# leoelm/Bayesian_inference_for_NN

Measured on AMD Instinct MI355X. Metric: posterior samples/sec (grad-steps/sec) on MLP 784->200->10, batch 1024, higher is better.
Workload: dtype f32; 1 GPU; SGLD, MLP 784->200->10 (D=159010), synthetic MNIST-shaped 48000x784 fp32 resident in HBM, batch 1024 (last batch of an epoch 896), 1 chain per GPU, device-resident run replayed from hipGraphs; seed=2024, parallelism=independent chains x1 (replicas only, no data-path collective)

## Files before the change

bayesian_inference_for_nn_amd/csrc/pyz_api.hip:

```cpp

#include <algorithm>
#include <cmath>
#include <cstring>

#include "pyz_common.h"
#include "pyz_fused.h"
#include "pyz_gemm.h"
#include "pyz_gemm_ring.h"
#include "pyz_hmc_fused.h"
#include "pyz_hmc_multi.h"
#include "pyz_input_grad.h"
#include "pyz_kernels.h"
#include "pyz_predict_moments.h"
#include "pyz_rng.h"
#include "pyz_sgld_chains.h"

namespace {

inline hipStream_t as_stream(void *s) { return reinterpret_cast<hipStream_t>(s); }
inline int cdiv(long long a, long long b) { return (int)((a + b - 1) / b); }

int ensure_bytes(void **ptr, size_t *cap, size_t need, pyz_mlp *m) {
  if (*cap >= need) return PYZ_OK;
  if (*ptr) PYZ_HIP(hipFree(*ptr));
  *ptr = nullptr;
  *cap = 0;
  PYZ_HIP(hipMalloc(ptr, need));
  m->ws_bytes += need;
  *cap = need;
  return PYZ_OK;
}

struct Extra {
  size_t grad_cap = 0, grad2_cap = 0, qsave_cap = 0, part_cap = 0, part2_cap = 0, scal_cap = 0;
// ... 321 lines not shown
    g.ctl = ctl;
    pyz_launch_bwd_data(g, grid_batch, P, st);
  }
}

inline int wgrad_tiles(const pyz_mlp *m) {
  int tiles = 0;
  for (int l = 0; l < m->L; ++l) tiles += ((m->dims[l] + 1 + 31) / 32) * ((m->dims[l + 1] + 31) / 32);
  return tiles;
}

int wgrad_layers(pyz_mlp *m, int P, const float *x, const int32_t *row_idx, const StepCtl *ctl, WgradArgs &a,
                 const float *gathered) {
  int tiles = 0;
  a.L = m->L;
  for (int l = 0; l < m->L; ++l) {
    WgradLayer &ly = a.lay[l];
    ly.K = m->dims[l];
    ly.N = m->dims[l + 1];
    if (l == 0) {
      ly.in = (row_idx && gathered) ? gathered : x;
      ly.in_pstride = 0;
      ly.gather = (row_idx && !gathered) ? 1 : 0;
    } else {
      ly.in = m->act[l - 1];
      ly.in_pstride = (long long)m->max_batch * ly.K;
      ly.gather = 0;
    }
    ly.lda = ly.K;
    ly.delta = m->delta[l];
    ly.delta_pstride = (long long)m->max_batch * ly.N;
    ly.w_off = m->w_off[l];
    ly.tile0 = tiles;
    tiles += ((ly.K + 1 + 31) / 32) * ((ly.N + 31) / 32);
  }
  a.row_idx = row_idx;
  a.ctl = ctl;
  a.part = m->part;
  a.nblk = m->cur_nblk;
  a.tiles = tiles;
  a.nonfinite = m->nonfinite;
  a.wt = pyz_wt_for(P);
  return tiles;
}

void launch_wgrad_all(pyz_mlp *m, int P, const float *x, const int32_t *row_idx, int grid_batch, const StepCtl *ctl,
                      WgradArgs &a, hipStream_t st, const float *gathered) {
  const int tiles = wgrad_layers(m, P, x, row_idx, ctl, a, gathered);
  const int S = pyz_pick_waves((long long)tiles * P, (grid_batch + 1) / 2);
  dim3 grid(pyz_pad8((long long)tiles + 1, P), P);
  if (a.prep.src && P == 1) grid.x = (unsigned)(tiles + 1 + std::max(pyz_cu_count() - tiles - 1, 24));
  switch (S) {
    case 1:
      if (a.mode == PYZ_UPD_NONE) PYZ_LAUNCH((k_wgrad_all<1, true>), grid, dim3(64), 0, st, a);
      else PYZ_LAUNCH(k_wgrad_all<1>, grid, dim3(64), 0, st, a);
      break;
    case 2: PYZ_LAUNCH(k_wgrad_all<2>, grid, dim3(128), 2 * 4096, st, a); break;
    case 4: PYZ_LAUNCH(k_wgrad_all<4>, grid, dim3(256), 4 * 4096, st, a); break;
    case 8: PYZ_LAUNCH(k_wgrad_all<8>, grid, dim3(512), 8 * 4096, st, a); break;
    default: PYZ_LAUNCH(k_wgrad_all<16>, grid, dim3(1024), 16 * 4096, st, a); break;
  }
}

void launch_wgrad_adam(pyz_mlp *m, const float *x, const int32_t *row_idx, int grid_batch, const StepCtl *ctl, AdamArgs &a,
                       hipStream_t st, const float *gathered) {
  const int tiles = wgrad_layers(m, 1, x, row_idx, ctl, a.w, gathered);
  const int S = pyz_pick_waves(tiles, (grid_batch + 1) / 2);
  const dim3 grid(tiles + 1);
// ... 2367 lines not shown
```

bayesian_inference_for_nn_amd/csrc/pyz_common.h:

```cpp
#pragma once

#include <hip/hip_runtime.h>
#include <hip/hip_ext.h>

#include <cstdarg>
#include <cstdint>
#include <cstdio>
#include <string>
#include <vector>

#include "../../include/pyz.h"

#define PYZ_MAX_LAYERS 16

typedef float f32x16 __attribute__((ext_vector_type(16)));
typedef float f32x4 __attribute__((ext_vector_type(4)));

struct StepCtl {
  int32_t batch;
  float lr;
  long long n;
  long long row_off;
  int32_t i;
  int32_t slot0;
// ... 2 lines not shown

#ifdef PYZ_STAMPS
#define PYZ_STAMP_KERNELS 6
#define PYZ_STAMP_BLOCKS 256
#define PYZ_STAMP_WAVES 16
#define PYZ_STAMP_SLOTS 8
__device__ unsigned long long pyz_dbg_buf[PYZ_STAMP_KERNELS][PYZ_STAMP_BLOCKS][PYZ_STAMP_WAVES][PYZ_STAMP_SLOTS][2];
#define PYZ_STAMP(kid, slot)                                                                   \
  do {                                                                                         \
    __builtin_amdgcn_sched_barrier(0);                                                         \
    if ((threadIdx.x & 63) == 0 && blockIdx.x < PYZ_STAMP_BLOCKS && blockIdx.y == 0) {        \
      unsigned long long t0_, t1_;                                                             \
      asm volatile("s_memtime %0\n\ts_memrealtime %1\n\ts_waitcnt lgkmcnt(0)" : "=s"(t0_), "=s"(t1_)::"memory"); \
      pyz_dbg_buf[kid][blockIdx.x][threadIdx.x >> 6][slot][0] = t0_;                          \
      pyz_dbg_buf[kid][blockIdx.x][threadIdx.x >> 6][slot][1] = t1_;                          \
    }                                                                                          \
    __builtin_amdgcn_sched_barrier(0);                                                         \
  } while (0)
#define PYZ_LAP(lap, slot)                                                                   \
  do {                                                                                       \
    __builtin_amdgcn_sched_barrier(0);                                                       \
    unsigned long long t_;                                                                   \
    asm volatile("s_memtime %0\n\ts_waitcnt lgkmcnt(0)" : "=s"(t_)::"memory");              \
    (lap)[slot] += t_ - (lap)[15];                                                           \
    (lap)[15] = t_;                                                                          \
    __builtin_amdgcn_sched_barrier(0);                                                       \
  } while (0)
#else
#define PYZ_STAMP(kid, slot)
#define PYZ_LAP(lap, slot)
#endif

__device__ __forceinline__ int pyz_wave_id() { return __builtin_amdgcn_readfirstlane((int)(threadIdx.x >> 6)); }

__device__ __forceinline__ StepCtl pyz_ctl_first(const StepCtl *ctl, const StepCtl &init, const int on) {
  if (on && blockIdx.x == 0 && blockIdx.y == 0 && threadIdx.x == 0) *const_cast<StepCtl *>(ctl) = init;
  int ib = init.batch, ii = init.i, is0 = init.slot0, inr = init.n_run;
  float il = init.lr;
  long long in_ = init.n, iro = init.row_off;
  asm volatile("" : "+s"(ib), "+s"(ii), "+s"(is0), "+s"(il), "+s"(in_), "+s"(iro), "+s"(inr));
  StepCtl c;
  c.batch = on ? ib : ctl->batch;
  c.lr = on ? il : ctl->lr;
  c.n = on ? in_ : ctl->n;
  c.row_off = on ? iro : ctl->row_off;
  c.i = on ? ii : ctl->i;
  c.slot0 = on ? is0 : ctl->slot0;
  c.n_run = on ? inr : ctl->n_run;
  return c;
}

__device__ __forceinline__ void pyz_st(float *p, const float v, const int wt) {
  if (wt)
    asm volatile("global_store_dword %0, %1, off sc1" ::"v"(p), "v"(v) : "memory");
  else
    *p = v;
}

inline std::string &pyz_err_slot() {
  static thread_local std::string s;
  return s;
}

inline int pyz_fail(int code, const char *fmt, ...) {
  char buf[512];
  va_list ap;
// ... 147 lines not shown
```

bayesian_inference_for_nn_amd/csrc/pyz_fused.h:

```cpp
#pragma once

#include <type_traits>

#include "pyz_common.h"
#include "pyz_gemm.h"
#include "pyz_kernels.h"

struct HeadArgs {
  const float *hin;
  long long hin_pstride;
  int lda;
  const int32_t *row_idx;
  int gather_hin;
  const float *theta;
  long long theta_pstride;
  long long w_off;
  int K, N;
  int loss, act_last, act_prev, vec;
  const void *y;
  float *out_last;
  float *delta_last;
  float *delta_prev;
  long long last_pstride, prev_pstride;
  double *part;
  int nblk;
  const StepCtl *ctl;
  StepCtl init;
  int init_on;
  int wt;
  const StepCtl *gate;
  int gate_mod;
  const float *hparts;
  int n_hparts;
  long long hpart_stride;
  const float *bias_prev;
  float *h_store;
};

__device__ __forceinline__ float pyz_grp8_max(float v) {
  v = fmaxf(v, __shfl_xor(v, 1, 64));
  v = fmaxf(v, __shfl_xor(v, 2, 64));
  return fmaxf(v, __shfl_xor(v, 4, 64));
}
__device__ __forceinline__ float pyz_grp8_sum(float v) {
  v += __shfl_xor(v, 1, 64);
  v += __shfl_xor(v, 2, 64);
  return v + __shfl_xor(v, 4, 64);
}

__global__ void __launch_bounds__(512) k_head(HeadArgs g) {
  extern __shared__ float lds[];
  PYZ_STAMP(1, 0);
  const int S = blockDim.x >> 6, w = pyz_wave_id(), l = threadIdx.x & 63, r = l & 31, h = l >> 5;
  if (g.gate && g.gate->n % g.gate_mod == 0) return;
  float *red = lds, *zt = lds + S * 1024, *dt = zt + 32 * 33;
  double *lsum = reinterpret_cast<double *>(dt + 32 * 33);
  const StepCtl ctl = pyz_ctl_first(g.ctl, g.init, g.init_on);
  const int batch = ctl.batch, p = blockIdx.y, m0 = blockIdx.x * 32;
  if (m0 >= batch) {
    if (threadIdx.x == 0) g.part[p * g.nblk + blockIdx.x] = 0.0;
    return;
  }
  const int K = g.K, N = g.N;
  const int32_t *idx = g.row_idx ? g.row_idx + ctl.row_off : nullptr;
// ... 179 lines not shown
  return v;
}

__device__ __forceinline__ float pyz_row16_allmax(float v) {
  v = fmaxf(v, pyz_dpp<0xB1>(v));
  v = fmaxf(v, pyz_dpp<0x4E>(v));
  v = fmaxf(v, pyz_dpp<0x141>(v));
  v = fmaxf(v, pyz_dpp<0x140>(v));
  return v;
}

template <int UT, int NP>
struct PyzHeadW {
  float wv[UT][NP];
  float bias_mine;
};

template <int UT, int NP>
__device__ __forceinline__ void pyz_head_load_w(const HeadArgs &g, const int p, const int l, PyzHeadW<UT, NP> &W) {
  const int K = g.K, N = g.N;
  const float *wl = g.theta + p * g.theta_pstride + g.w_off;
  const __amdgpu_buffer_rsrc_t rw = __builtin_amdgcn_make_buffer_rsrc(const_cast<float *>(wl), 0, (K + 1) * N * 4, 0x00020000);
  constexpr unsigned OOB = 0x7FFFFF00u;
#pragma unroll
  for (int t = 0; t < UT; ++t) {
    const int u = l + 64 * t;
    const unsigned wo = u < K ? 4u * (unsigned)u * (unsigned)N : OOB;
#pragma unroll
    for (int c = 0; c < NP; ++c) W.wv[t][c] = pyz_buf_load(rw, wo + 4u * (unsigned)c, 0u);
  }
  W.bias_mine = pyz_buf_load(rw, l < N ? 4u * ((unsigned)K * (unsigned)N + (unsigned)l) : OOB, 0u);
}

template <int UT, int NP, bool PRELOADED, bool HP = false>
__device__ __forceinline__ void pyz_head_row(const HeadArgs &g, const int batch, const long long row_off, const int p,
                                             const int m, const int l, PyzHeadW<UT, NP> &W) {
  const int K = g.K, N = g.N;
  long long yrow = m;
  if (g.row_idx) yrow = g.row_idx[row_off + m];
  const float *hp = g.hin + p * g.hin_pstride + (g.gather_hin ? yrow : (long long)m) * g.lda;
  const __amdgpu_buffer_rsrc_t rh = __builtin_amdgcn_make_buffer_rsrc(const_cast<float *>(hp), 0, K * 4, 0x00020000);
  float hv[UT], z[NP];
  if constexpr (HP) {
    const float *pp = g.hparts + (long long)m * K;
    const __amdgpu_buffer_rsrc_t rp = __builtin_amdgcn_make_buffer_rsrc(const_cast<float *>(pp), 0,
        (int)(((long long)(g.n_hparts - 1) * g.hpart_stride + K) * 4), 0x00020000);
    const __amdgpu_buffer_rsrc_t rb = __builtin_amdgcn_make_buffer_rsrc(const_cast<float *>(g.bias_prev), 0, K * 4, 0x00020000);
    constexpr unsigned OOBH = 0x7FFFFF00u;
    float pv[UT][8], bv[UT];
#pragma unroll
    for (int t = 0; t < UT; ++t) {
      const int u = l + 64 * t;
#pragma unroll
      for (int sp = 0; sp < 8; ++sp)
        pv[t][sp] = pyz_buf_load(rp, (u < K && sp < g.n_hparts) ? 4u * (unsigned)(sp * g.hpart_stride + u) : OOBH, 0u);
      bv[t] = pyz_buf_load(rb, 4u * (unsigned)u, 0u);
    }
#pragma unroll
    for (int t = 0; t < UT; ++t) {
      float a = pv[t][0];
#pragma unroll
      for (int sp = 1; sp < 8; ++sp) a += pv[t][sp];
      hv[t] = pyz_act(a + bv[t], g.act_prev);
      const int u = l + 64 * t;
      if (u < K) pyz_st(g.h_store + (long long)m * K + u, hv[t], g.wt);
    }
  } else {
#pragma unroll
    for (int t = 0; t < UT; ++t) hv[t] = pyz_buf_load(rh, 4u * (unsigned)(l + 64 * t), 0u);
  }
  if (!PRELOADED) pyz_head_load_w<UT, NP>(g, p, l, W);
  const auto &wv = W.wv;
  const float bias_mine = W.bias_mine;
  int ylab = 0;
  if (g.loss == PYZ_LOSS_SCCE) ylab = reinterpret_cast<const int32_t *>(g.y)[yrow];
  PYZ_STAMP(1, 1);
#pragma unroll
  for (int c = 0; c < NP; ++c) {
    float a = 0.0f;
#pragma unroll
    for (int t = 0; t < UT; ++t) a = fmaf(hv[t], wv[t][c], a);
    z[c] = a;
  }
#pragma unroll
  for (int c = 0; c < NP; ++c) {
    const float v = pyz_row16_allsum(z[c]);
    z[c] = ((pyz_readlane(v, 0) + pyz_readlane(v, 16)) + (pyz_readlane(v, 32) + pyz_readlane(v, 48))) + pyz_readlane(bias_mine, c);
  }
  PYZ_STAMP(1, 2);
  float d2[NP], lm, my_d = 0.0f, my_o = 0.0f;
  if (g.loss == PYZ_LOSS_SCCE && NP <= 16) {
    const int lc = l & 15;
    float zc = z[0];
#pragma unroll
    for (int c = 1; c < NP; ++c) zc = (lc == c) ? z[c] : zc;
    const bool on = lc < N;
    const float mx = pyz_row16_allmax(on ? zc : -3.0e38f);
    const float exv = on ? expf(zc - mx) : 0.0f;
    const float se = pyz_row16_allsum(exv);
    const float lse = mx + logf(se);
    const bool mine = on && lc == ylab;
    float zy = pyz_row16_allsum(mine ? zc : 0.0f);
    zy = (ylab >= 0 && ylab < N) ? zy : __builtin_nanf("");
    const float inv = 1.0f / (float)batch, rse = 1.0f / se;
    my_d = (exv * rse - (mine ? 1.0f : 0.0f)) * inv;
    my_o = zc;
// ... 48 lines not shown
      lm = a / (float)N;
    }
#pragma unroll
    for (int c = 0; c < NP; ++c) {
      my_d = (l == c) ? d2[c] : my_d;
      my_o = (l == c) ? outv[c] : my_o;
    }
  }
  PYZ_STAMP(1, 3);
  if (l < N) {
    if (g.out_last) pyz_st(g.out_last + p * g.last_pstride + (long long)m * N + l, my_o, g.wt);
    if (g.delta_last) pyz_st(g.delta_last + p * g.last_pstride + (long long)m * N + l, my_d, g.wt);
  }
  if (l == 0) g.part[p * g.nblk + m] = (double)lm;
  PYZ_STAMP(1, 4);
  if (!g.delta_prev) return;
  float *op = g.delta_prev + p * g.prev_pstride + (long long)m * K;
  const int actp = g.act_prev;
#pragma unroll
  for (int t = 0; t < UT; ++t) {
    const int u = l + 64 * t;
    float a = 0.0f;
#pragma unroll
    for (int c = 0; c < NP; ++c) a = fmaf(d2[c], wv[t][c], a);
    if (u < K) pyz_st(op + u, a * pyz_act_grad(hv[t], actp), g.wt);
  }
  PYZ_STAMP(1, 5);
}

template <int UT, int NP, int RW = 1, bool HP = false>
__global__ void __launch_bounds__(256) k_head_rows(HeadArgs g) {
  PYZ_STAMP(1, 0);
  const int w = pyz_wave_id(), l = threadIdx.x & 63;
  if (g.gate && g.gate->n % g.gate_mod == 0) return;
  const StepCtl ctl = pyz_ctl_first(g.ctl, g.init, g.init_on);
  const int batch = ctl.batch, p = blockIdx.y;
  const int m0 = (blockIdx.x * 4 + w) * RW;
  if (m0 >= batch) {
    if (l < RW && m0 + l < g.nblk) g.part[p * g.nblk + m0 + l] = 0.0;
    return;
  }
  PyzHeadW<UT, NP> W;
  if (RW == 1) {
    pyz_head_row<UT, NP, false, HP>(g, batch, ctl.row_off, p, m0, l, W);
    return;
  }
  pyz_head_load_w<UT, NP>(g, p, l, W);
#pragma unroll 1
  for (int rr = 0; rr < RW; ++rr) {
    const int m = m0 + rr;
    if (m >= batch) {
      if (l == 0 && m < g.nblk) g.part[p * g.nblk + m] = 0.0;
      continue;
    }
    pyz_head_row<UT, NP, true>(g, batch, ctl.row_off, p, m, l, W);
  }
}

struct PrepArgs {
  const float *src;
  float *dst;
  const int32_t *row_idx;
  const int32_t *tab_bs;
  long long row_stride;
  int K, lda;
  int fwd_tiles, fwd_tiles_n;
};

// ... 85 lines not shown
      tab_bc[e] = b.bc[e];
    }
    if (e == 0) {
      ctl->batch = t.bs[0];
      ctl->lr = t.lr[0];
      ctl->n = n;
      ctl->row_off = row_off;
      ctl->i = 0;
      ctl->slot0 = slot0;
      ctl->n_run = t.n - 1;
    }
  }
  pyz_prep_rows(g, g.row_idx + row_off, t.bs[0], (int)blockIdx.x, (int)gridDim.x, (int)blockIdx.x);
}

struct WgradLayer {
  const float *in;
  long long in_pstride;
  const float *delta;
  long long delta_pstride;
  long long w_off;
  int lda, K, N;
  int tile0;
  int gather;
};

#define PYZ_UPD_NONE 0
#define PYZ_UPD_SGD 1
#define PYZ_UPD_SGLD 2
#define PYZ_UPD_BBB 3
#define PYZ_UPD_SWAG 4

struct WgradArgs {
  WgradLayer lay[PYZ_MAX_LAYERS];
  int L;
  int tiles;
  const int32_t *row_idx;
  const StepCtl *ctl;
  int mode;
  float *grad;
  long long grad_pstride;
  float *theta, *mean, *sq_mean;
  uint64_t seed;
  const float *unit_noise;
  float *dev_row;
  int swag_update;
  int swag_freq, swag_k;
  float *dev_base;
  long long dev_stride;
  float alpha, prior_mean, prior_rho, bbb_lr;
  const float *pm_vec, *pr_vec;
  uint32_t bbb_step;
  int bbb_chained;
  const double *part_kl;
  int nblk_kl;
  float *cost;
  float *w_next;
  double *part_kl_next;
  const double *part;
  int nblk;
  float *loss;
  int loss_indexed;
  StepCtl *next;
  const int32_t *tab_bs;
  const float *tab_lr;
  long long row_stride;
  int *nonfinite;
  float *ploss;
  int wt;
  PrepArgs prep;
};

struct PyzUpdOut {
  float th, mu, sq, dev;
  bool wr_mu, wr_sq, wr_dev;
  float *dev_row;
};

__device__ __forceinline__ PyzUpdOut pyz_update_math(const WgradArgs &g, const int mode, const long long e, const float gv,
                                                     const float th0, const float mu0, const float sq0, const float zz,
                                                     const float lr, const long long nstep) {
  PyzUpdOut o;
  o.th = o.mu = o.sq = o.dev = 0.0f;
  o.wr_mu = o.wr_sq = o.wr_dev = false;
  o.dev_row = nullptr;
  if (mode == PYZ_UPD_SGD) {
    o.th = th0 - lr * gv;
  } else if (mode == PYZ_UPD_SWAG) {
    const float th = th0 - lr * gv;
    o.th = th;
    const bool upd = g.swag_freq > 0 ? (nstep % g.swag_freq == 0) : (g.swag_update != 0);
    if (upd) {
      const float fn = (float)nstep, fn1 = fn + 1.0f;
      o.mu = (mu0 * fn + th) / fn1;
      o.sq = (sq0 * fn + th * th) / fn1;
      o.dev = th - o.mu;
      o.wr_mu = o.wr_sq = true;
      o.dev_row = g.swag_freq > 0
                      ? g.dev_base + min((nstep + g.swag_freq - 1) / g.swag_freq, (long long)g.swag_k - 1) * g.dev_stride
                      : g.dev_row;
      o.wr_dev = o.dev_row != nullptr;
    }
  } else if (mode == PYZ_UPD_BBB) {
    const float pmean = g.pm_vec ? g.pm_vec[e] : g.prior_mean;
    const float sp = pyz_softplus(g.pr_vec ? g.pr_vec[e] : g.prior_rho), isp2 = 1.0f / (sp * sp);
    const float mu = th0, rho = mu0, wv = sq0;
    const float sg = pyz_softplus(rho), sig = pyz_sigmoid(rho);
    const float d = wv - mu, is2 = 1.0f / (sg * sg);
    const float g_mu = g.alpha * d * is2;
    const float g_rho = g.alpha * (-1.0f / sg + d * d * is2 / sg) * sig;
    const float g_w = gv + g.alpha * (-d * is2 + (wv - pmean) * isp2);
    const float blr = g.bbb_chained ? lr : g.bbb_lr;
    o.th = mu - blr * (g_mu + g_w);
    o.mu = rho - blr * (zz * sig * g_w + g_rho);
    o.wr_mu = true;
  } else if (mode == PYZ_UPD_SGLD) {
    const float fn = (float)nstep, fn1 = fn + 1.0f;
    const float noise = lr * zz;
    const float th = th0 + (-lr) * (gv + noise);
    o.th = th;
    o.mu = (mu0 * fn + th) / fn1;
    o.sq = (sq0 * fn + th * th) / fn1;
    o.wr_mu = o.wr_sq = true;
  }
  return o;
}

__device__ __forceinline__ void pyz_update_store(const WgradArgs &g, const int mode, const long long e, const int p,
                                                 const float gv, const PyzUpdOut &o) {
  if (mode == PYZ_UPD_NONE) {
    g.grad[p * g.grad_pstride + e] = gv;
    return;
  }
  pyz_st(g.theta + e, o.th, g.wt);
  if (o.wr_mu) pyz_st(g.mean + e, o.mu, g.wt);
  if (o.wr_sq) pyz_st(g.sq_mean + e, o.sq, g.wt);
  if (o.wr_dev) o.dev_row[e] = o.dev;
}

__device__ __forceinline__ void pyz_step_duties(const WgradArgs &g, const int l) {
  const int batch = g.ctl->batch;
  if (g.loss) {
    const double v = pyz_sum_partials(g.part, g.nblk);
    if (l == 0) {
      float *lo = g.loss + (g.loss_indexed ? g.ctl->slot0 + g.ctl->i : 0);
      lo[0] = (float)(v / (double)batch);
      pyz_note_loss(g.nonfinite, lo[0]);
      if (g.next) pyz_prepare_next(g.ctl, g.next, g.tab_bs, g.tab_lr, g.row_stride);
    }
  }
  if (g.mode == PYZ_UPD_BBB) {
    const double v = pyz_sum_partials(g.part, g.nblk), k = pyz_sum_partials(g.part_kl, g.nblk_kl);
    if (l == 0) {
      const float loss = (float)(v / (double)batch), kl = (float)k;
      float *co = g.cost + (g.bbb_chained ? 4 * (g.ctl->slot0 + g.ctl->i) : 0);
// ... 6 lines not shown
  }
}


template <class H>
__device__ __forceinline__ void pyz_wgrad_accumulate(f32x16 &acc, const float *abase, const int ic, const float *dbase,
                                                     const int n, const int lda, const int N, const int batch, int s,
                                                     const int se, const int h, const bool is_w, const bool is_b, H hook) {
  const float bconst = is_b ? 1.0f : 0.0f;
  const unsigned a_lane = ((unsigned)h * (unsigned)lda + (unsigned)ic) * 4u;
  const unsigned d_lane = ((unsigned)h * (unsigned)N + (unsigned)n) * 4u;
  const unsigned a_row2 = 8u * (unsigned)lda, d_row2 = 8u * (unsigned)N;
  const __amdgpu_buffer_rsrc_t ra =
      __builtin_amdgcn_make_buffer_rsrc(const_cast<float *>(abase), 0, (int)((unsigned)batch * (unsigned)lda * 4u), 0x00020000);
  const __amdgpu_buffer_rsrc_t rd =
      __builtin_amdgcn_make_buffer_rsrc(const_cast<float *>(dbase), 0, (int)((unsigned)batch * (unsigned)N * 4u), 0x00020000);
  const int full = batch >> 1;
  pyz_steps1_all(
      s, min(se, full), acc,
      [&](int st, float &a, float &d) {
        a = pyz_buf_load(ra, a_lane, (unsigned)PYZ_HOT(st, batch) * a_row2);
        d = pyz_buf_load(rd, d_lane, (unsigned)PYZ_HOT(st, batch) * d_row2);
      },
      [&](int, float &a, float &) { a = is_w ? a : bconst; }, hook);
  if (se > full) {
    const int b = batch - 1;
    float a = abase[(size_t)b * lda + ic], d = dbase[(size_t)b * N + n];
    a = h == 0 ? (is_w ? a : bconst) : 0.0f;
    d = h == 0 ? d : 0.0f;
    acc = pyz_mfma(a, d, acc);
  }
}

template <int S, bool PLAIN = false>
__global__ void __launch_bounds__(64 * S) k_wgrad_all(WgradArgs g) {
  extern __shared__ float red[];
  PYZ_STAMP(2, 0);
  constexpr int EPT = 16 / S;
  const int w = pyz_wave_id(), l = threadIdx.x & 63;
  const int r = l & 31, h = l >> 5;
  if (blockIdx.x >= (unsigned)g.tiles) {
    if (blockIdx.x == (unsigned)g.tiles && blockIdx.y == 0 && w == 0) pyz_step_duties(g, l);
    if (blockIdx.x == (unsigned)g.tiles && w == 0 && g.ploss) {
      const double tot = pyz_sum_partials(g.part + (long long)blockIdx.y * g.nblk, g.nblk);
      if (l == 0) {
        g.ploss[blockIdx.y] = (float)(tot / (double)g.ctl->batch);
        pyz_note_loss(g.nonfinite, g.ploss[blockIdx.y]);
      }
    }
    if (!PLAIN && blockIdx.x > (unsigned)g.tiles && blockIdx.y == 0 && g.prep.src) {
      const int i2 = g.ctl->i + 1;
      if (i2 < g.ctl->n_run)
        pyz_prep_rows(g.prep, g.prep.row_idx + g.ctl->row_off + g.prep.row_stride, g.prep.tab_bs[i2],
                      (int)blockIdx.x - g.tiles - 1, (int)gridDim.x - g.tiles - 1, (int)blockIdx.x);
      PYZ_STAMP(2, 3);
    }
    return;
  }
  const int tile = pyz_xcd_remap(blockIdx.x, g.tiles);
  int li = 0;
  while (li + 1 < g.L && tile >= g.lay[li + 1].tile0) ++li;
  const WgradLayer &ly = g.lay[li];
  const int batch = g.ctl->batch;
  const int K = ly.K, N = ly.N;
  const int tiles_n = (N + 31) >> 5;
  const int t = tile - ly.tile0;
  const int i0 = (t / tiles_n) * 32, n0 = (t % tiles_n) * 32;
  const int p = blockIdx.y;
  const long long w_off = ly.w_off;
  const int mode = PLAIN ? PYZ_UPD_NONE : g.mode;
  const long long nstep = g.ctl->n;
  const float lr = g.ctl->lr;

  long long ee[EPT];
  bool ev[EPT];
  float th0[PLAIN ? 1 : EPT], mu0[PLAIN ? 1 : EPT], sq0[PLAIN ? 1 : EPT], zz[PLAIN ? 1 : EPT];
  float zg[PLAIN ? 1 : EPT];
  float zn[PLAIN ? 1 : EPT];
  const bool fuse_next = !PLAIN && mode == PYZ_UPD_BBB && g.w_next != nullptr;
  auto prefetch = [&]() {
#pragma unroll
    for (int q = 0; q < EPT; ++q) {
      int ro, co;
      if (S == 1) {
        ro = (q & 3) + 8 * (q >> 2) + 4 * h;
        co = r;
      } else {
        const int e = threadIdx.x + q * 64 * S;
        ro = e >> 5;
        co = e & 31;
      }
      const int ii = i0 + ro, nn = n0 + co;
      ev[q] = ii <= K && nn < N;
      ee[q] = w_off + (long long)min(ii, K) * N + min(nn, N - 1);
      if (PLAIN) continue;
      th0[q] = mu0[q] = sq0[q] = zz[q] = zg[q] = 0.0f;
      if (mode != PYZ_UPD_NONE) th0[q] = g.theta[ee[q]];
      if (mode == PYZ_UPD_SGLD || mode == PYZ_UPD_BBB || mode == PYZ_UPD_SWAG) {
        mu0[q] = g.mean[ee[q]];
        sq0[q] = g.sq_mean[ee[q]];
        if (g.unit_noise && mode != PYZ_UPD_SWAG) zz[q] = g.unit_noise[ee[q]];
      }
    }
    if (!PLAIN && (mode == PYZ_UPD_SGLD || mode == PYZ_UPD_BBB) && !g.unit_noise) {
#pragma unroll
      for (int q = 0; q < EPT; ++q) {
        zg[q] = mode == PYZ_UPD_SGLD ? pyz_normal1(g.seed, PYZ_STREAM_SGLD, (uint32_t)nstep, (uint64_t)ee[q])
                                     : pyz_normal1(g.seed, PYZ_STREAM_BBB, g.bbb_chained ? (uint32_t)nstep : g.bbb_step, (uint64_t)ee[q]);
      }
    }
    if (!PLAIN && fuse_next) {
#pragma unroll
      for (int q = 0; q < EPT; ++q) zn[q] = pyz_normal1(g.seed, PYZ_STREAM_BBB, (uint32_t)(nstep + 1), (uint64_t)ee[q]);
    }
  };

  const int i = i0 + r, n = min(n0 + r, N - 1);
  const int ic = min(i, K - 1);
  const bool is_w = i < K, is_b = i == K;
  const float *ap = ly.in + p * ly.in_pstride + ic;
  const float *dp = ly.delta + p * ly.delta_pstride + n;
  const int32_t *idx = (ly.gather && g.row_idx) ? g.row_idx + g.ctl->row_off : nullptr;
  f32x16 acc = {0};
  const int steps = (batch + 1) >> 1;
  int s = (steps * w) / S;
  const int se = (steps * (w + 1)) / S;
  PYZ_STAMP(2, 1);
  if (idx) {
    prefetch();
    for (int s0 = s; s0 < se; s0 += 32) {
      const int idxv = idx[min(2 * s0 + l, batch - 1)];
      const int lda = ly.lda;
      pyz_steps1_all(
          s0, min(s0 + 32, se), acc,
          [&](int st, float &a, float &d) {
            const int bc = PYZ_HOT(min(2 * st + h, batch - 1), batch);
            const long long row = PYZ_HOT(__shfl(idxv, 2 * (st - s0) + h, 64), batch);
            a = ap[row * lda];
            d = dp[(long long)bc * N];
          },
          [&](int st, float &a, float &d) {
            const bool vb = 2 * st + h < batch;
            a = vb ? (is_w ? a : (is_b ? 1.0f : 0.0f)) : 0.0f;
            d = vb ? d : 0.0f;
          });
    }
  } else {
    pyz_wgrad_accumulate(acc, ly.in + p * ly.in_pstride, ic, ly.delta + p * ly.delta_pstride, n, ly.lda, N, batch, s, se, h,
                         is_w, is_b, prefetch);
  }
  PYZ_STAMP(2, 2);
  float gv[EPT];
  if (S == 1) {
#pragma unroll
    for (int q = 0; q < EPT; ++q) gv[q] = acc[q];
// ... 29 lines not shown
                                        PLAIN ? 0.0f : (g.unit_noise ? zz[q] : zg[q]), lr, nstep);
    pyz_update_store(g, mode, ee[q], p, gv[q], o);
    if (fuse_next) {
      const long long e = ee[q];
      const float pmean = g.pm_vec ? g.pm_vec[e] : g.prior_mean;
      float sp = sp_s, lsp = lsp_s;
      if (g.pr_vec) {
        sp = pyz_softplus(g.pr_vec[e]);
        lsp = logf(sp);
      }
      const float mu = o.th, sg = pyz_softplus(o.mu);
      const float wn = zn[q] * sg + mu;
      pyz_st(g.w_next + e, wn, g.wt);
      const float a = (wn - mu) / sg, b = (wn - pmean) / sp;
      const float lq = -0.5f * a * a - logf(sg) - PYZ_LOG_SQRT_2PI;
      const float lp = -0.5f * b * b - lsp - PYZ_LOG_SQRT_2PI;
      klp += (double)lq - (double)lp;
    }
  }
  if (!PLAIN && fuse_next) {
    double tot = pyz_wave_sum(klp);
    if (S > 1) {
      double *sm = reinterpret_cast<double *>(red);
      __syncthreads();
      if (l == 0) sm[w] = tot;
      __syncthreads();
      tot = 0.0;
      if (threadIdx.x == 0)
        for (int ww = 0; ww < S; ++ww) tot += sm[ww];
    }
    if (threadIdx.x == 0) g.part_kl_next[blockIdx.x] = tot;
  }
  PYZ_STAMP(2, 3);
}

template <class H>
__device__ __forceinline__ void pyz_wgrad_accumulate_sq(f32x16 &acc, f32x16 &acc2, const float fb, const float *abase,
                                                        const int ic, const float *dbase, const int n, const int lda,
                                                        const int N, const int batch, int s, const int se, const int h,
                                                        const bool is_w, const bool is_b, H hook) {
  const float bconst = is_b ? 1.0f : 0.0f;
  const unsigned a_lane = ((unsigned)h * (unsigned)lda + (unsigned)ic) * 4u;
  const unsigned d_lane = ((unsigned)h * (unsigned)N + (unsigned)n) * 4u;
  const unsigned a_row2 = 8u * (unsigned)lda, d_row2 = 8u * (unsigned)N;
  const __amdgpu_buffer_rsrc_t ra =
      __builtin_amdgcn_make_buffer_rsrc(const_cast<float *>(abase), 0, (int)((unsigned)batch * (unsigned)lda * 4u), 0x00020000);
  const __amdgpu_buffer_rsrc_t rd =
      __builtin_amdgcn_make_buffer_rsrc(const_cast<float *>(dbase), 0, (int)((unsigned)batch * (unsigned)N * 4u), 0x00020000);
  const int full = batch >> 1;
  pyz_steps1_all(
      s, min(se, full), acc,
      [&](int st, float &a, float &d) {
        a = pyz_buf_load(ra, a_lane, (unsigned)PYZ_HOT(st, batch) * a_row2);
        d = pyz_buf_load(rd, d_lane, (unsigned)PYZ_HOT(st, batch) * d_row2);
      },
      [&](int, float &a, float &d) {
        a = is_w ? a : bconst;
        const float gd = d * fb;
        acc2 = pyz_mfma(a * a, gd * gd, acc2);
      },
      hook);
  if (se > full) {
    const int b = batch - 1;
    float a = abase[(size_t)b * lda + ic], d = dbase[(size_t)b * N + n];
    a = h == 0 ? (is_w ? a : bconst) : 0.0f;
    d = h == 0 ? d : 0.0f;
// ... 349 lines not shown
```

bayesian_inference_for_nn_amd/csrc/pyz_gemm.h:

```cpp
#pragma once

#include <cstdlib>

#include "pyz_common.h"

struct DenseArgs {
  const float *in;
  long long in_pstride;
  int lda;
  const float *theta;
  long long theta_pstride;
  long long w_off;
  int K, N;
  float *out;
  long long out_pstride;
  const float *aux;
  long long aux_pstride;
  int act;
  int vec;
  const StepCtl *ctl;
  const int32_t *row_idx;
  float *gather_out;
  StepCtl init;
  int init_on;
  int wt;
  int rows_cap;
  int n_part, grid_rows;
  int n_cgrp, cgrp_w;
  int k_split;
  float *part_out;
  long long part_stride;
  const StepCtl *gate;
  int gate_mod;
};

__device__ __forceinline__ int pyz_xcd_remap(const int bid, const int n) {
  const int q = n >> 3, r = n & 7, x = bid & 7, local = bid >> 3;
  return (x < r ? x * (q + 1) : r * (q + 1) + (x - r) * q) + local;
}

#ifdef PYZ_EXP_HOT
#define PYZ_HOT(v, batch) ((v) & ((batch) < 0 ? -1 : 0))
#else
#define PYZ_HOT(v, batch) (v)
#endif

__device__ __forceinline__ f32x16 pyz_mfma(float a, float b, f32x16 c) {
#ifdef PYZ_EXP_NOMFMA
  c[0] += a * b;
  return c;
#else
  return __builtin_amdgcn_mfma_f32_32x32x2f32(a, b, c, 0, 0, 0);
#endif
}

__device__ __forceinline__ float pyz_act(float z, int act) {
  switch (act) {
    case PYZ_ACT_RELU: return z < 0.0f ? 0.0f : z;
    case PYZ_ACT_TANH: return tanhf(z);
    case PYZ_ACT_SIGMOID: return 1.0f / (1.0f + expf(-z));
    default: return z;
  }
}

__device__ __forceinline__ float pyz_act_grad(float h, int act) {
  switch (act) {
    case PYZ_ACT_RELU: return h > 0.0f ? 1.0f : 0.0f;
    case PYZ_ACT_TANH: return 1.0f - h * h;
    case PYZ_ACT_SIGMOID: return h * (1.0f - h);
    default: return 1.0f;
  }
}

__device__ __forceinline__ float pyz_bce_row(float z, float y, float &p) {
  const float e = expf(-fabsf(z));
  const float r = 1.0f / (1.0f + e);
  p = z >= 0.0f ? r : (z < 0.0f ? e * r : z);
  const float u = 1.0f + e;
  const float l1p = u == 1.0f ? e : logf(u) * (e / (u - 1.0f));
  return fmaxf(z, 0.0f) - z * y + l1p;
}

template <class F>
__device__ __forceinline__ void pyz_tile_epilogue(const f32x16 &acc, float *red, F store) {
  const int S = blockDim.x >> 6, w = pyz_wave_id(), l = threadIdx.x & 63;
  const int r = l & 31, h = l >> 5;
  if (S == 1) {
#pragma unroll
    for (int i = 0; i < 16; ++i) store((i & 3) + 8 * (i >> 2) + 4 * h, r, acc[i]);
    return;
  }
  float *my = red + w * 1024;
#pragma unroll
  for (int i = 0; i < 16; ++i) my[((i & 3) + 8 * (i >> 2) + 4 * h) * 32 + r] = acc[i];
  __syncthreads();
  for (int e = threadIdx.x; e < 1024; e += blockDim.x) {
    float s = red[e];
    for (int ww = 1; ww < S; ++ww) s += red[ww * 1024 + e];
    store(e >> 5, e & 31, s);
  }
}

struct PyzNoFix {
  __device__ __forceinline__ void operator()(int, float &, float &) const {}
};

struct PyzNoHook {
  __device__ __forceinline__ void operator()() const {}
};

template <int G, class L, class F, class H = PyzNoHook>
__device__ __forceinline__ void pyz_pipe1(int s, const int se, f32x16 &acc, L load, F fix, H hook = H()) {
  if (s >= se) {
    hook();
    return;
  }
  float an[G], bn[G], a[G], b[G];
  const int last = se - 1;
#pragma unroll
  for (int u = 0; u < G; ++u) load(min(s + u, last), an[u], bn[u]);
  __builtin_amdgcn_sched_barrier(0);
  hook();
  __builtin_amdgcn_sched_barrier(0);
  for (;;) {
#pragma unroll
    for (int u = 0; u < G; ++u) {
      a[u] = an[u];
      b[u] = bn[u];
    }
    const int sn = s + G;
    if (sn < se) {
#pragma unroll
// ... 102 lines not shown
          *reinterpret_cast<float4 *>(gp + 8 * c + 4 * h) = a4;
#endif
        }
      },
      hook);
  const int t0 = 8 * c8, steps = (K - t0 + 1) >> 1;
  const unsigned vt = (unsigned)h * N4 + n4;
  pyz_steps1_all(
      0, (steps - w + S - 1) / S, acc,
      [&](int u, float &a, float &b) {
        const int kb = t0 + 2 * (w + S * u);
        const int kk = kb + h;
        a = ap[kk < K ? kk : 0];
        b = pyz_buf_load(rw, vt, (unsigned)kb * N4);
      },
      [&](int u, float &a, float &b) {
        const int kk = t0 + 2 * (w + S * u) + h;
        const bool vk = kk < K;
        if (gp && vk && copy_rem == 0) gp[kk] = a;
        a = vk ? a : 0.0f;
        b = vk ? b : 0.0f;
      });
  if (w == 0) {
    acc = pyz_mfma(h == 0 ? 1.0f : 0.0f, h == 0 ? bias : 0.0f, acc);
  }
}

__global__ void k_dense_fwd(DenseArgs g) {
  extern __shared__ float red[];
  PYZ_STAMP(0, 0);
  const int S = blockDim.x >> 6, w = pyz_wave_id(), l = threadIdx.x & 63;
  const int r = l & 31, h = l >> 5;
  const int tiles_n = (g.N + 31) >> 5;
  if (g.gate && g.gate->n % g.gate_mod == 0) return;
  const int tile = pyz_xcd_remap(blockIdx.x, gridDim.x);
  const int m0 = (tile / tiles_n) * 32, n0 = (tile % tiles_n) * 32;
  int cap = g.rows_cap;
  long long row_off = 0;
  if (cap <= 0) {
    asm volatile("; the step scalars are needed here" ::: "memory");
    const StepCtl ctl = pyz_ctl_first(g.ctl, g.init, g.init_on);
    cap = __builtin_amdgcn_readfirstlane(ctl.batch);
    row_off = ctl.row_off;
  }
  if (m0 >= cap) return;
  const int p = blockIdx.y;
  const int K = g.K, N = g.N;
  const int m = min(m0 + r, cap - 1), n = min(n0 + r, N - 1);
  long long row = m;
  if (g.row_idx) row = g.row_idx[row_off + m];
  const float *ap = g.in + p * g.in_pstride + row * g.lda;
  const float *wl = g.theta + p * g.theta_pstride + g.w_off;
  f32x16 acc = {0};
  PYZ_STAMP(0, 1);
  float *gp = (g.gather_out && p == 0) ? g.gather_out + (long long)m * K : nullptr;
  int batch = 0;
  const int32_t *ctl_batch = &g.ctl->batch;
  pyz_fwd_accumulate(acc, ap, wl, n, K, N, g.vec, w, S, h, gp, tiles_n, tile % tiles_n,
                     [&]() { batch = __hip_atomic_load(ctl_batch, __ATOMIC_RELAXED, __HIP_MEMORY_SCOPE_AGENT); });
  batch = g.rows_cap > 0 ? __builtin_amdgcn_readfirstlane(batch) : cap;
  PYZ_STAMP(0, 2);
  float *op = g.out + p * g.out_pstride;
  const int act = g.act, wt = g.wt;
  pyz_tile_epilogue(acc, red, [&](int ro, int co, float v) {
    const int mm = m0 + ro, nn = n0 + co;
    if (mm < batch && nn < N) pyz_st(op + (long long)mm * N + nn, pyz_act(v, act), wt);
// ... 372 lines not shown
```

Baseline: 40500 grad-steps/s.

## Reorder kernel arg structs and batch scalar loads to cut kernel prologue latency

Reorders the fields of HeadArgs, DenseArgs and WgradArgs so the hot fields sit together, and uses asm constraints so the compiler issues all kernel-argument scalar loads in one batch at kernel entry. Step-control scalars are now loaded as vector loads and broadcast with readfirstlane. The wgrad layer lookup becomes a branchless compare over a per-layer tile0 table. The update mode is made a template parameter, and the multi-wave tile reduction is unrolled per wave count. These target the fixed prologue and serialized-load latency of small kernels replayed from graphs. The cost is more template instantiations and code size, and some update arithmetic now uses explicit FMAs, which slightly changes rounding.

```diff
diff --git a/bayesian_inference_for_nn_amd/csrc/pyz_api.hip b/bayesian_inference_for_nn_amd/csrc/pyz_api.hip
--- a/bayesian_inference_for_nn_amd/csrc/pyz_api.hip
+++ b/bayesian_inference_for_nn_amd/csrc/pyz_api.hip
@@ -1,5 +1,6 @@
 
 #include <algorithm>
+#include <climits>
 #include <cmath>
 #include <cstring>
 
@@ -387,8 +388,10 @@
     ly.delta_pstride = (long long)m->max_batch * ly.N;
     ly.w_off = m->w_off[l];
     ly.tile0 = tiles;
+    a.tile0[l] = tiles;
     tiles += ((ly.K + 1 + 31) / 32) * ((ly.N + 31) / 32);
   }
+  for (int l = m->L; l < PYZ_MAX_LAYERS; ++l) a.tile0[l] = INT_MAX;
   a.row_idx = row_idx;
   a.ctl = ctl;
   a.part = m->part;
diff --git a/bayesian_inference_for_nn_amd/csrc/pyz_common.h b/bayesian_inference_for_nn_amd/csrc/pyz_common.h
--- a/bayesian_inference_for_nn_amd/csrc/pyz_common.h
+++ b/bayesian_inference_for_nn_amd/csrc/pyz_common.h
@@ -58,6 +58,35 @@
 #endif
 
 __device__ __forceinline__ int pyz_wave_id() { return __builtin_amdgcn_readfirstlane((int)(threadIdx.x >> 6)); }
+
+
+struct PyzCtlHot {
+  int batch;
+  float lr;
+  long long n, row_off;
+};
+__device__ __forceinline__ PyzCtlHot pyz_ctl_request(const StepCtl *ctl) {
+  PyzCtlHot c;
+  c.batch = ctl->batch;
+  c.lr = ctl->lr;
+  c.n = ctl->n;
+  c.row_off = ctl->row_off;
+  return c;
+}
+__device__ __forceinline__ PyzCtlHot pyz_ctl_arrived(const PyzCtlHot &raw) {
+  int b = raw.batch;
+  float lr = raw.lr;
+  long long n = raw.n, ro = raw.row_off;
+  asm volatile("; step scalars" : "+v"(b), "+v"(lr), "+v"(n), "+v"(ro));
+  PyzCtlHot c;
+  c.batch = __builtin_amdgcn_readfirstlane(b);
+  c.lr = __builtin_bit_cast(float, __builtin_amdgcn_readfirstlane(__builtin_bit_cast(int, lr)));
+  const unsigned nl = __builtin_amdgcn_readfirstlane((int)(unsigned)n), nh = __builtin_amdgcn_readfirstlane((int)(n >> 32));
+  const unsigned rl = __builtin_amdgcn_readfirstlane((int)(unsigned)ro), rh = __builtin_amdgcn_readfirstlane((int)(ro >> 32));
+  c.n = (long long)(((unsigned long long)nh << 32) | nl);
+  c.row_off = (long long)(((unsigned long long)rh << 32) | rl);
+  return c;
+}
 
 __device__ __forceinline__ StepCtl pyz_ctl_first(const StepCtl *ctl, const StepCtl &init, const int on) {
   if (on && blockIdx.x == 0 && blockIdx.y == 0 && threadIdx.x == 0) *const_cast<StepCtl *>(ctl) = init;
diff --git a/bayesian_inference_for_nn_amd/csrc/pyz_fused.h b/bayesian_inference_for_nn_amd/csrc/pyz_fused.h
--- a/bayesian_inference_for_nn_amd/csrc/pyz_fused.h
+++ b/bayesian_inference_for_nn_amd/csrc/pyz_fused.h
@@ -9,27 +9,28 @@
 struct HeadArgs {
   const float *hin;
   long long hin_pstride;
-  int lda;
-  const int32_t *row_idx;
-  int gather_hin;
   const float *theta;
   long long theta_pstride;
   long long w_off;
+  const StepCtl *ctl;
+  const int32_t *row_idx;
+  const StepCtl *gate;
+  const void *y;
+  double *part;
+  int lda;
   int K, N;
-  int loss, act_last, act_prev, vec;
-  const void *y;
+  int loss;
+  int gather_hin;
+  int gate_mod;
+  int init_on;
+  int nblk;
+  int act_last, act_prev, vec;
+  int wt;
   float *out_last;
   float *delta_last;
   float *delta_prev;
   long long last_pstride, prev_pstride;
-  double *part;
-  int nblk;
-  const StepCtl *ctl;
   StepCtl init;
-  int init_on;
-  int wt;
-  const StepCtl *gate;
-  int gate_mod;
   const float *hparts;
   int n_hparts;
   long long hpart_stride;
@@ -275,14 +276,20 @@
   W.bias_mine = pyz_buf_load(rw, l < N ? 4u * ((unsigned)K * (unsigned)N + (unsigned)l) : OOB, 0u);
 }
 
+template <int UT>
+__device__ __forceinline__ void pyz_head_load_h(const HeadArgs &g, const int p, const long long hrow, const int l, float (&hv)[UT]) {
+  const float *hp = g.hin + p * g.hin_pstride + hrow * g.lda;
+  const __amdgpu_buffer_rsrc_t rh = __builtin_amdgcn_make_buffer_rsrc(const_cast<float *>(hp), 0, g.K * 4, 0x00020000);
+#pragma unroll
+  for (int t = 0; t < UT; ++t) hv[t] = pyz_buf_load(rh, 4u * (unsigned)(l + 64 * t), 0u);
+}
+
 template <int UT, int NP, bool PRELOADED, bool HP = false>
 __device__ __forceinline__ void pyz_head_row(const HeadArgs &g, const int batch, const long long row_off, const int p,
                                              const int m, const int l, PyzHeadW<UT, NP> &W) {
   const int K = g.K, N = g.N;
-  long long yrow = m;
-  if (g.row_idx) yrow = g.row_idx[row_off + m];
-  const float *hp = g.hin + p * g.hin_pstride + (g.gather_hin ? yrow : (long long)m) * g.lda;
-  const __amdgpu_buffer_rsrc_t rh = __builtin_amdgcn_make_buffer_rsrc(const_cast<float *>(hp), 0, K * 4, 0x00020000);
+  int yidx = m;
+  if (g.row_idx) yidx = g.row_idx[row_off + m];
   float hv[UT], z[NP];
   if constexpr (HP) {
     const float *pp = g.hparts + (long long)m * K;
@@ -309,12 +316,18 @@
       if (u < K) pyz_st(g.h_store + (long long)m * K + u, hv[t], g.wt);
     }
   } else {
-#pragma unroll
-    for (int t = 0; t < UT; ++t) hv[t] = pyz_buf_load(rh, 4u * (unsigned)(l + 64 * t), 0u);
+    if (g.gather_hin) {
+      asm volatile("; gathered input: the row index is needed here" ::: "memory");
+      pyz_head_load_h<UT>(g, p, __builtin_amdgcn_readfirstlane(yidx), l, hv);
+    } else {
+      pyz_head_load_h<UT>(g, p, m, l, hv);
+    }
   }
   if (!PRELOADED) pyz_head_load_w<UT, NP>(g, p, l, W);
   const auto &wv = W.wv;
   const float bias_mine = W.bias_mine;
+  asm volatile("; the row index arrives here" : "+v"(yidx));
+  const long long yrow = yidx;
   int ylab = 0;
   if (g.loss == PYZ_LOSS_SCCE) ylab = reinterpret_cast<const int32_t *>(g.y)[yrow];
   PYZ_STAMP(1, 1);
@@ -429,8 +442,20 @@
 __global__ void __launch_bounds__(256) k_head_rows(HeadArgs g) {
   PYZ_STAMP(1, 0);
   const int w = pyz_wave_id(), l = threadIdx.x & 63;
+  asm volatile("; arguments in one trip" ::"s"(g.hin), "s"(g.hin_pstride), "s"(g.theta), "s"(g.theta_pstride), "s"(g.w_off),
+               "s"(g.ctl), "s"(g.row_idx), "s"(g.gate), "s"(g.y), "s"(g.part), "s"(g.lda), "s"(g.K), "s"(g.N), "s"(g.loss),
+               "s"(g.gather_hin), "s"(g.gate_mod), "s"(g.init_on), "s"(g.nblk), "s"(g.act_last), "s"(g.act_prev), "s"(g.vec),
+               "s"(g.wt));
   if (g.gate && g.gate->n % g.gate_mod == 0) return;
-  const StepCtl ctl = pyz_ctl_first(g.ctl, g.init, g.init_on);
+  StepCtl ctl;
+  if (g.init_on) {
+    asm volatile("; the step scalars by value" ::: "memory");
+    ctl = pyz_ctl_first(g.ctl, g.init, 1);
+  } else {
+    const PyzCtlHot c = pyz_ctl_arrived(pyz_ctl_request(g.ctl));
+    ctl.batch = c.batch;
+    ctl.row_off = c.row_off;
+  }
   const int batch = ctl.batch, p = blockIdx.y;
   const int m0 = (blockIdx.x * 4 + w) * RW;
   if (m0 >= batch) {
@@ -582,17 +607,27 @@
 #define PYZ_UPD_SWAG 4
 
 struct WgradArgs {
+  int tiles;
+  int L;
+  int mode;
+  int wt;
+  const StepCtl *ctl;
+  const int32_t *row_idx;
+  float *theta, *mean, *sq_mean;
+  const float *unit_noise;
+  uint64_t seed;
+  int tile0[PYZ_MAX_LAYERS];
+  const double *part;
+  int nblk;
+  int loss_indexed;
+  float *loss;
+  StepCtl *next;
+  const int32_t *tab_bs;
+  const float *tab_lr;
+  int *nonfinite;
   WgradLayer lay[PYZ_MAX_LAYERS];
-  int L;
-  int tiles;
-  const int32_t *row_idx;
-  const StepCtl *ctl;
-  int mode;
   float *grad;
   long long grad_pstride;
-  float *theta, *mean, *sq_mean;
-  uint64_t seed;
-  const float *unit_noise;
   float *dev_row;
   int swag_update;
   int swag_freq, swag_k;
@@ -607,19 +642,12 @@
   float *cost;
   float *w_next;
   double *part_kl_next;
-  const double *part;
-  int nblk;
-  float *loss;
-  int loss_indexed;
-  StepCtl *next;
-  const int32_t *tab_bs;
-  const float *tab_lr;
   long long row_stride;
-  int *nonfinite;
   float *ploss;
-  int wt;
   PrepArgs prep;
 };
+
+static_assert(offsetof(WgradArgs, lay) % 64 == 0 && sizeof(WgradLayer) == 64, "a layer's entry is one 64-byte line");
 
 struct PyzUpdOut {
   float th, mu, sq, dev;
@@ -635,15 +663,16 @@
   o.wr_mu = o.wr_sq = o.wr_dev = false;
   o.dev_row = nullptr;
   if (mode == PYZ_UPD_SGD) {
-    o.th = th0 - lr * gv;
+    o.th = __builtin_fmaf(-lr, gv, th0);
   } else if (mode == PYZ_UPD_SWAG) {
-    const float th = th0 - lr * gv;
+#pragma clang fp contract(off)
+    const float th = __builtin_fmaf(-lr, gv, th0);
     o.th = th;
     const bool upd = g.swag_freq > 0 ? (nstep % g.swag_freq == 0) : (g.swag_update != 0);
     if (upd) {
       const float fn = (float)nstep, fn1 = fn + 1.0f;
       o.mu = (mu0 * fn + th) / fn1;
-      o.sq = (sq0 * fn + th * th) / fn1;
+      o.sq = __builtin_fmaf(th, th, sq0 * fn) / fn1;
       o.dev = th - o.mu;
       o.wr_mu = o.wr_sq = true;
       o.dev_row = g.swag_freq > 0
@@ -665,12 +694,13 @@
     o.mu = rho - blr * (zz * sig * g_w + g_rho);
     o.wr_mu = true;
   } else if (mode == PYZ_UPD_SGLD) {
+#pragma clang fp contract(off)
     const float fn = (float)nstep, fn1 = fn + 1.0f;
-    const float noise = lr * zz;
-    const float th = th0 + (-lr) * (gv + noise);
+    const float gn = __builtin_fmaf(lr, zz, gv);
+    const float th = __builtin_fmaf(-lr, gn, th0);
     o.th = th;
     o.mu = (mu0 * fn + th) / fn1;
-    o.sq = (sq0 * fn + th * th) / fn1;
+    o.sq = __builtin_fmaf(th, th, sq0 * fn) / fn1;
     o.wr_mu = o.wr_sq = true;
   }
   return o;
@@ -743,45 +773,31 @@
   }
 }
 
-template <int S, bool PLAIN = false>
-__global__ void __launch_bounds__(64 * S) k_wgrad_all(WgradArgs g) {
-  extern __shared__ float red[];
-  PYZ_STAMP(2, 0);
+template <int S, bool PLAIN, int MODE>
+__device__ __forceinline__ void pyz_wgrad_tile(const WgradArgs &g, float *red) {
   constexpr int EPT = 16 / S;
   const int w = pyz_wave_id(), l = threadIdx.x & 63;
   const int r = l & 31, h = l >> 5;
-  if (blockIdx.x >= (unsigned)g.tiles) {
-    if (blockIdx.x == (unsigned)g.tiles && blockIdx.y == 0 && w == 0) pyz_step_duties(g, l);
-    if (blockIdx.x == (unsigned)g.tiles && w == 0 && g.ploss) {
-      const double tot = pyz_sum_partials(g.part + (long long)blockIdx.y * g.nblk, g.nblk);
-      if (l == 0) {
-        g.ploss[blockIdx.y] = (float)(tot / (double)g.ctl->batch);
-        pyz_note_loss(g.nonfinite, g.ploss[blockIdx.y]);
-      }
-    }
-    if (!PLAIN && blockIdx.x > (unsigned)g.tiles && blockIdx.y == 0 && g.prep.src) {
-      const int i2 = g.ctl->i + 1;
-      if (i2 < g.ctl->n_run)
-        pyz_prep_rows(g.prep, g.prep.row_idx + g.ctl->row_off + g.prep.row_stride, g.prep.tab_bs[i2],
-                      (int)blockIdx.x - g.tiles - 1, (int)gridDim.x - g.tiles - 1, (int)blockIdx.x);
-      PYZ_STAMP(2, 3);
-    }
-    return;
-  }
   const int tile = pyz_xcd_remap(blockIdx.x, g.tiles);
   int li = 0;
-  while (li + 1 < g.L && tile >= g.lay[li + 1].tile0) ++li;
+#pragma unroll
+  for (int j = 1; j < PYZ_MAX_LAYERS; ++j) li += tile >= g.tile0[j] ? 1 : 0;
+  li = __builtin_amdgcn_readfirstlane(li);
   const WgradLayer &ly = g.lay[li];
-  const int batch = g.ctl->batch;
+  const PyzCtlHot ctl_raw = pyz_ctl_request(g.ctl);
+  asm volatile("; the layer in one trip" ::"s"(ly.in), "s"(ly.in_pstride), "s"(ly.delta), "s"(ly.delta_pstride), "s"(ly.w_off),
+               "s"(ly.lda), "s"(ly.K), "s"(ly.N), "s"(ly.tile0), "s"(ly.gather));
+  const PyzCtlHot ctl = pyz_ctl_arrived(ctl_raw);
+  const int batch = ctl.batch;
   const int K = ly.K, N = ly.N;
   const int tiles_n = (N + 31) >> 5;
   const int t = tile - ly.tile0;
   const int i0 = (t / tiles_n) * 32, n0 = (t % tiles_n) * 32;
   const int p = blockIdx.y;
   const long long w_off = ly.w_off;
-  const int mode = PLAIN ? PYZ_UPD_NONE : g.mode;
-  const long long nstep = g.ctl->n;
-  const float lr = g.ctl->lr;
+  constexpr int mode = PLAIN ? PYZ_UPD_NONE : MODE;
+  const long long nstep = ctl.n;
+  const float lr = ctl.lr;
 
   long long ee[EPT];
   bool ev[EPT];
@@ -831,7 +847,7 @@
   const bool is_w = i < K, is_b = i == K;
   const float *ap = ly.in + p * ly.in_pstride + ic;
   const float *dp = ly.delta + p * ly.delta_pstride + n;
-  const int32_t *idx = (ly.gather && g.row_idx) ? g.row_idx + g.ctl->row_off : nullptr;
+  const int32_t *idx = (ly.gather && g.row_idx) ? g.row_idx + ctl.row_off : nullptr;
   f32x16 acc = {0};
   const int steps = (batch + 1) >> 1;
   int s = (steps * w) / S;
@@ -927,6 +943,46 @@
     if (threadIdx.x == 0) g.part_kl_next[blockIdx.x] = tot;
   }
   PYZ_STAMP(2, 3);
+}
+
+template <int S, bool PLAIN = false>
+__global__ void __launch_bounds__(64 * S) k_wgrad_all(WgradArgs g) {
+  extern __shared__ float red[];
+  PYZ_STAMP(2, 0);
+  const int w = pyz_wave_id(), l = threadIdx.x & 63;
+  asm volatile("; arguments in one trip" ::"s"(g.tiles), "s"(g.mode), "s"(g.ctl), "s"(g.row_idx), "s"(g.tile0[1]),
+               "s"(g.tile0[2]), "s"(g.tile0[3]), "s"(g.tile0[4]), "s"(g.tile0[5]), "s"(g.tile0[6]), "s"(g.tile0[7]),
+               "s"(g.tile0[8]), "s"(g.tile0[9]), "s"(g.tile0[10]), "s"(g.tile0[11]), "s"(g.tile0[12]), "s"(g.tile0[13]),
+               "s"(g.tile0[14]), "s"(g.tile0[15]));
+  if (blockIdx.x >= (unsigned)g.tiles) {
+    if (blockIdx.x == (unsigned)g.tiles && blockIdx.y == 0 && w == 0) pyz_step_duties(g, l);
+    if (blockIdx.x == (unsigned)g.tiles && w == 0 && g.ploss) {
+      const double tot = pyz_sum_partials(g.part + (long long)blockIdx.y * g.nblk, g.nblk);
+      if (l == 0) {
+        g.ploss[blockIdx.y] = (float)(tot / (double)g.ctl->batch);
+        pyz_note_loss(g.nonfinite, g.ploss[blockIdx.y]);
+      }
+    }
+    if (!PLAIN && blockIdx.x > (unsigned)g.tiles && blockIdx.y == 0 && g.prep.src) {
+      const int i2 = g.ctl->i + 1;
+      if (i2 < g.ctl->n_run)
+        pyz_prep_rows(g.prep, g.prep.row_idx + g.ctl->row_off + g.prep.row_stride, g.prep.tab_bs[i2],
+                      (int)blockIdx.x - g.tiles - 1, (int)gridDim.x - g.tiles - 1, (int)blockIdx.x);
+      PYZ_STAMP(2, 3);
+    }
+    return;
+  }
+  if constexpr (PLAIN) {
+    pyz_wgrad_tile<S, true, PYZ_UPD_NONE>(g, red);
+  } else {
+    switch (g.mode) {
+      case PYZ_UPD_SGLD: pyz_wgrad_tile<S, false, PYZ_UPD_SGLD>(g, red); break;
+      case PYZ_UPD_SGD: pyz_wgrad_tile<S, false, PYZ_UPD_SGD>(g, red); break;
+      case PYZ_UPD_SWAG: pyz_wgrad_tile<S, false, PYZ_UPD_SWAG>(g, red); break;
+      case PYZ_UPD_BBB: pyz_wgrad_tile<S, false, PYZ_UPD_BBB>(g, red); break;
+      default: pyz_wgrad_tile<S, false, PYZ_UPD_NONE>(g, red); break;
+    }
+  }
 }
 
 template <class H>
diff --git a/bayesian_inference_for_nn_amd/csrc/pyz_gemm.h b/bayesian_inference_for_nn_amd/csrc/pyz_gemm.h
--- a/bayesian_inference_for_nn_amd/csrc/pyz_gemm.h
+++ b/bayesian_inference_for_nn_amd/csrc/pyz_gemm.h
@@ -7,31 +7,31 @@
 struct DenseArgs {
   const float *in;
   long long in_pstride;
-  int lda;
   const float *theta;
   long long theta_pstride;
   long long w_off;
+  int lda;
   int K, N;
+  int vec;
+  int rows_cap;
+  int gate_mod;
   float *out;
   long long out_pstride;
-  const float *aux;
-  long long aux_pstride;
-  int act;
-  int vec;
   const StepCtl *ctl;
   const int32_t *row_idx;
   float *gather_out;
+  const StepCtl *gate;
+  int act;
+  int wt;
+  int init_on;
+  const float *aux;
+  long long aux_pstride;
   StepCtl init;
-  int init_on;
-  int wt;
-  int rows_cap;
   int n_part, grid_rows;
   int n_cgrp, cgrp_w;
   int k_split;
   float *part_out;
   long long part_stride;
-  const StepCtl *gate;
-  int gate_mod;
 };
 
 __device__ __forceinline__ int pyz_xcd_remap(const int bid, const int n) {
@@ -81,6 +81,24 @@
   return fmaxf(z, 0.0f) - z * y + l1p;
 }
 
+template <int S, class F>
+__device__ __forceinline__ void pyz_tile_combine(const float *red, F &store) {
+  constexpr int EPT = 16 / S;
+  float v[EPT][S];
+#pragma unroll
+  for (int q = 0; q < EPT; ++q)
+#pragma unroll
+    for (int ww = 0; ww < S; ++ww) v[q][ww] = red[ww * 1024 + (int)threadIdx.x + q * 64 * S];
+#pragma unroll
+  for (int q = 0; q < EPT; ++q) {
+    const int e = (int)threadIdx.x + q * 64 * S;
+    float s = v[q][0];
+#pragma unroll
+    for (int ww = 1; ww < S; ++ww) s += v[q][ww];
+    store(e >> 5, e & 31, s);
+  }
+}
+
 template <class F>
 __device__ __forceinline__ void pyz_tile_epilogue(const f32x16 &acc, float *red, F store) {
   const int S = blockDim.x >> 6, w = pyz_wave_id(), l = threadIdx.x & 63;
@@ -94,10 +112,12 @@
 #pragma unroll
   for (int i = 0; i < 16; ++i) my[((i & 3) + 8 * (i >> 2) + 4 * h) * 32 + r] = acc[i];
   __syncthreads();
-  for (int e = threadIdx.x; e < 1024; e += blockDim.x) {
-    float s = red[e];
-    for (int ww = 1; ww < S; ++ww) s += red[ww * 1024 + e];
-    store(e >> 5, e & 31, s);
+  switch (S) {
+    case 2: pyz_tile_combine<2>(red, store); break;
+    case 4: pyz_tile_combine<4>(red, store); break;
+    case 8: pyz_tile_combine<8>(red, store); break;
+    case 16: pyz_tile_combine<16>(red, store); break;
+    default: __builtin_trap();
   }
 }
 
@@ -266,6 +286,10 @@
   const int S = blockDim.x >> 6, w = pyz_wave_id(), l = threadIdx.x & 63;
   const int r = l & 31, h = l >> 5;
   const int tiles_n = (g.N + 31) >> 5;
+  asm volatile("; arguments in one trip" ::"s"(g.in), "s"(g.in_pstride), "s"(g.theta), "s"(g.theta_pstride), "s"(g.w_off),
+               "s"(g.lda), "s"(g.K), "s"(g.N), "s"(g.vec), "s"(g.rows_cap), "s"(g.gate_mod), "s"(g.out), "s"(g.out_pstride),
+               "s"(g.ctl), "s"(g.row_idx), "s"(g.gather_out), "s"(g.gate), "s"(g.act), "s"(g.wt), "s"((int)gridDim.x),
+               "s"((int)blockDim.x));
   if (g.gate && g.gate->n % g.gate_mod == 0) return;
   const int tile = pyz_xcd_remap(blockIdx.x, gridDim.x);
   const int m0 = (tile / tiles_n) * 32, n0 = (tile % tiles_n) * 32;
```

Result: faster. 42540 grad-steps/s, median of 6 (+5.0%).
